# coreperf/rejit

Hardware: AMD Instinct MI355X
Metric: GB/s text scanned (regexdna 9 patterns, 50M-line input); matches/s alongside (higher is better)
Workload: dtype u8

## Files before the change

rejit_amd/csrc/plane_count.hip:

```cpp
#include <hip/hip_runtime.h>
#include <hip/hip_ext.h>

#include <cstdlib>

#include "exact_count.h"
#include "kernels.h"
#include "short_walk.h"
#include "stream_load.h"

namespace rejit_amd {

namespace {

constexpr int kWave = 64;
constexpr uint64_t kBlock = 2048;
constexpr uint32_t kPieceB = 1024;
constexpr uint32_t kStashWords = (2048 + 16) / 4;
#ifndef RJ_PC_RING
#define RJ_PC_RING 256
#endif
constexpr uint32_t kRing = RJ_PC_RING;

__device__ __forceinline__ int lane_id() { return static_cast<int>(threadIdx.x) & (kWave - 1); }

__device__ __forceinline__ uint32_t lanes_below(uint64_t mask) {
  return __builtin_amdgcn_mbcnt_hi(static_cast<uint32_t>(mask >> 32), __builtin_amdgcn_mbcnt_lo(static_cast<uint32_t>(mask), 0u));
}

__device__ __forceinline__ uint32_t from_lane_above(uint32_t v, uint32_t last) {
  return static_cast<uint32_t>(__builtin_amdgcn_update_dpp(static_cast<int>(last), static_cast<int>(v), 0x130, 0xF, 0xF, false));
}
__device__ __forceinline__ uint32_t from_lane_below(uint32_t v, uint32_t first) {
  return static_cast<uint32_t>(__builtin_amdgcn_update_dpp(static_cast<int>(first), static_cast<int>(v), 0x138, 0xF, 0xF, false));
}

template <int CTRL, int ROW_MASK>
__device__ __forceinline__ uint32_t dpp_or_zero(uint32_t x) {
  return static_cast<uint32_t>(__builtin_amdgcn_update_dpp(0, static_cast<int>(x), CTRL, ROW_MASK, 0xF, true));
}
__device__ __forceinline__ uint32_t wave_inclusive_sum(uint32_t x) {
  x += dpp_or_zero<0x111, 0xF>(x);
  x += dpp_or_zero<0x112, 0xF>(x);
  x += dpp_or_zero<0x114, 0xF>(x);
  x += dpp_or_zero<0x118, 0xF>(x);
  x += dpp_or_zero<0x142, 0xA>(x);
  x += dpp_or_zero<0x143, 0xC>(x);
  return x;
}

struct Consts {
  uint32_t cmask;
  uint32_t shift;
};

__device__ __forceinline__ uint32_t codes4(uint32_t d, const Consts& k) { return __builtin_amdgcn_udot4(d & k.cmask, 0x40100401u, 0u, false); }

__device__ __forceinline__ uint32_t codes16(const uint4& v, const Consts& k) {
  const uint32_t s = k.shift;
  return (codes4(v.x, k) >> s) | (codes4(v.y, k) << (8 - s)) | (codes4(v.z, k) << (16 - s)) | (codes4(v.w, k) << (24 - s));
}

struct Raw {
  uint4 a, b;
};

__device__ __forceinline__ void load_block(const uint8_t* block, uint32_t lane_off, Raw& r) {
  r.a = stream_load16(block + lane_off);
  r.b = stream_load16(block + lane_off + kPieceB);
}

__device__ __forceinline__ uint32_t guarded_dword(const uint8_t* text, uint64_t n, uint64_t at) {
  uint32_t v = 0;
#pragma unroll
  for (int k = 0; k < 4; k++)
    if (at + k < n) v |= static_cast<uint32_t>(text[at + k]) << (8 * k);
  return v;
}

template <int NB>
__device__ __forceinline__ uint32_t plane_test(uint32_t ta, uint32_t tb, uint32_t ha, uint32_t hb, const PlaneCountParams& a) {
  constexpr uint32_t kEven = 0x55555555u;
  const uint32_t L = (ta & kEven) | ((tb << 1) & ~kEven);
  const uint32_t H = ((ta >> 1) & kEven) | (tb & ~kEven);
  const uint32_t Ln = (ha & kEven) | ((hb << 1) & ~kEven);
  const uint32_t Hn = ((ha >> 1) & kEven) | (hb & ~kEven);
  register uint32_t q0 asm("v48") = ~(L | H);
  register uint32_t q1 asm("v49") = L & ~H;
  register uint32_t q2 asm("v50") = ~L & H;
  register uint32_t q3 asm("v51") = L & H;
  register uint32_t n0 asm("v52") = ~(Ln | Hn);
  register uint32_t n1 asm("v53") = Ln & ~Hn;
  register uint32_t n2 asm("v54") = ~Ln & Hn;
  register uint32_t n3 asm("v55") = Ln & Hn;
  uint32_t codes = ~a.mask_bits;
  asm volatile("" : "+s"(codes));
  auto code = [&](int b, int i) { return (codes >> (16 * b + 2 * i)) & 3u; };
  uint32_t E[8][NB], Z[NB], O[NB];
#pragma unroll
  for (int half = 0; half < 2; half++) {
    if (NB == 1) {
      if (half == 0) {
      asm volatile(
          "s_set_gpr_idx_on %[c00], 0x3\n"
          "v_mov_b32 %[e00], v48\n"
          "s_set_gpr_idx_idx %[c10]\n"
          "v_alignbit_b32 %[e10], v52, v48, 2\n"
          "s_set_gpr_idx_idx %[c20]\n"
          "v_alignbit_b32 %[e20], v52, v48, 4\n"
          "s_set_gpr_idx_idx %[c30]\n"
          "v_alignbit_b32 %[e30], v52, v48, 6\n"
          "s_set_gpr_idx_off\n"
          : [e00] "=&v"(E[0][0]), [e10] "=&v"(E[1][0]), [e20] "=&v"(E[2][0]), [e30] "=&v"(E[3][0])
          : [c00] "s"(code(0, 0)), [c10] "s"(code(0, 1)), [c20] "s"(code(0, 2)), [c30] "s"(code(0, 3)), "v"(q0), "v"(q1), "v"(q2), "v"(q3), "v"(n0), "v"(n1), "v"(n2), "v"(n3));
      } else {
      asm volatile(
          "s_set_gpr_idx_on %[c40], 0x3\n"
          "v_alignbit_b32 %[e40], v52, v48, 8\n"
          "s_set_gpr_idx_idx %[c50]\n"
          "v_alignbit_b32 %[e50], v52, v48, 10\n"
          "s_set_gpr_idx_idx %[c60]\n"
          "v_alignbit_b32 %[e60], v52, v48, 12\n"
          "s_set_gpr_idx_idx %[c70]\n"
          "v_alignbit_b32 %[e70], v52, v48, 14\n"
          "s_set_gpr_idx_off\n"
          : [e40] "=&v"(E[4][0]), [e50] "=&v"(E[5][0]), [e60] "=&v"(E[6][0]), [e70] "=&v"(E[7][0])
          : [c40] "s"(code(0, 4)), [c50] "s"(code(0, 5)), [c60] "s"(code(0, 6)), [c70] "s"(code(0, 7)), "v"(q0), "v"(q1), "v"(q2), "v"(q3), "v"(n0), "v"(n1), "v"(n2), "v"(n3));
      }
    } else {
      if (half == 0) {
      asm volatile(
          "s_set_gpr_idx_on %[c00], 0x3\n"
          "v_mov_b32 %[e00], v48\n"
          "s_set_gpr_idx_idx %[c01]\n"
          "v_mov_b32 %[e01], v48\n"
          "s_set_gpr_idx_idx %[c10]\n"
          "v_alignbit_b32 %[e10], v52, v48, 2\n"
          "s_set_gpr_idx_idx %[c11]\n"
          "v_alignbit_b32 %[e11], v52, v48, 2\n"
          "s_set_gpr_idx_idx %[c20]\n"
          "v_alignbit_b32 %[e20], v52, v48, 4\n"
          "s_set_gpr_idx_idx %[c21]\n"
          "v_alignbit_b32 %[e21], v52, v48, 4\n"
          "s_set_gpr_idx_idx %[c30]\n"
          "v_alignbit_b32 %[e30], v52, v48, 6\n"
          "s_set_gpr_idx_idx %[c31]\n"
          "v_alignbit_b32 %[e31], v52, v48, 6\n"
          "s_set_gpr_idx_off\n"
          : [e00] "=&v"(E[0][0]), [e01] "=&v"(E[0][1]), [e10] "=&v"(E[1][0]), [e11] "=&v"(E[1][1]), [e20] "=&v"(E[2][0]), [e21] "=&v"(E[2][1]), [e30] "=&v"(E[3][0]), [e31] "=&v"(E[3][1])
          : [c00] "s"(code(0, 0)), [c01] "s"(code(1, 0)), [c10] "s"(code(0, 1)), [c11] "s"(code(1, 1)), [c20] "s"(code(0, 2)), [c21] "s"(code(1, 2)), [c30] "s"(code(0, 3)), [c31] "s"(code(1, 3)), "v"(q0), "v"(q1), "v"(q2), "v"(q3), "v"(n0), "v"(n1), "v"(n2), "v"(n3));
      } else {
      asm volatile(
          "s_set_gpr_idx_on %[c40], 0x3\n"
          "v_alignbit_b32 %[e40], v52, v48, 8\n"
          "s_set_gpr_idx_idx %[c41]\n"
          "v_alignbit_b32 %[e41], v52, v48, 8\n"
          "s_set_gpr_idx_idx %[c50]\n"
          "v_alignbit_b32 %[e50], v52, v48, 10\n"
          "s_set_gpr_idx_idx %[c51]\n"
          "v_alignbit_b32 %[e51], v52, v48, 10\n"
          "s_set_gpr_idx_idx %[c60]\n"
          "v_alignbit_b32 %[e60], v52, v48, 12\n"
          "s_set_gpr_idx_idx %[c61]\n"
          "v_alignbit_b32 %[e61], v52, v48, 12\n"
          "s_set_gpr_idx_idx %[c70]\n"
          "v_alignbit_b32 %[e70], v52, v48, 14\n"
          "s_set_gpr_idx_idx %[c71]\n"
          "v_alignbit_b32 %[e71], v52, v48, 14\n"
          "s_set_gpr_idx_off\n"
          : [e40] "=&v"(E[4][0]), [e41] "=&v"(E[4][1]), [e50] "=&v"(E[5][0]), [e51] "=&v"(E[5][1]), [e60] "=&v"(E[6][0]), [e61] "=&v"(E[6][1]), [e70] "=&v"(E[7][0]), [e71] "=&v"(E[7][1])
          : [c40] "s"(code(0, 4)), [c41] "s"(code(1, 4)), [c50] "s"(code(0, 5)), [c51] "s"(code(1, 5)), [c60] "s"(code(0, 6)), [c61] "s"(code(1, 6)), [c70] "s"(code(0, 7)), [c71] "s"(code(1, 7)), "v"(q0), "v"(q1), "v"(q2), "v"(q3), "v"(n0), "v"(n1), "v"(n2), "v"(n3));
// ... 76 lines not shown

template <bool TOL>
__device__ __forceinline__ uint32_t general_test(uint32_t ta, uint32_t tb, uint32_t ha, uint32_t hb, const PlaneCountGParams& g) {
  constexpr uint32_t kEven = 0x55555555u;
  const uint32_t L = (ta & kEven) | ((tb << 1) & ~kEven);
  const uint32_t H = ((ta >> 1) & kEven) | (tb & ~kEven);
  const uint32_t Ln = (ha & kEven) | ((hb << 1) & ~kEven);
  const uint32_t Hn = ((ha >> 1) & kEven) | (hb & ~kEven);
  register uint32_t q0 asm("v48") = ~(L | H);
  register uint32_t q1 asm("v49") = L & ~H;
  register uint32_t q2 asm("v50") = ~L & H;
  register uint32_t q3 asm("v51") = L & H;
  register uint32_t q4 asm("v52") = ~0u;
  register uint32_t n0 asm("v56") = ~(Ln | Hn);
  register uint32_t n1 asm("v57") = Ln & ~Hn;
  register uint32_t n2 asm("v58") = ~Ln & Hn;
  register uint32_t n3 asm("v59") = Ln & Hn;
  register uint32_t n4 asm("v60") = ~0u;
  uint32_t c = 0;
#pragma clang loop unroll(disable)
  for (uint32_t b = 0; b < g.c.n_bases; b++) {
    const uint32_t* ix = g.idx[b];
    uint32_t e0, e1, e2, e3, e4, e5, e6, e7;
    asm volatile(
        "s_set_gpr_idx_on %[i0], 0x3\n"
        "v_mov_b32 %[e0], v48\n"
        "s_set_gpr_idx_idx %[i1]\n"
        "v_alignbit_b32 %[e1], v56, v48, 2\n"
        "s_set_gpr_idx_idx %[i2]\n"
        "v_alignbit_b32 %[e2], v56, v48, 4\n"
        "s_set_gpr_idx_idx %[i3]\n"
        "v_alignbit_b32 %[e3], v56, v48, 6\n"
        "s_set_gpr_idx_idx %[i4]\n"
        "v_alignbit_b32 %[e4], v56, v48, 8\n"
        "s_set_gpr_idx_idx %[i5]\n"
        "v_alignbit_b32 %[e5], v56, v48, 10\n"
        "s_set_gpr_idx_idx %[i6]\n"
        "v_alignbit_b32 %[e6], v56, v48, 12\n"
        "s_set_gpr_idx_idx %[i7]\n"
        "v_alignbit_b32 %[e7], v56, v48, 14\n"
        "s_set_gpr_idx_off\n"
        : [e0] "=&v"(e0), [e1] "=&v"(e1), [e2] "=&v"(e2), [e3] "=&v"(e3), [e4] "=&v"(e4), [e5] "=&v"(e5), [e6] "=&v"(e6), [e7] "=&v"(e7)
        : [i0] "s"(ix[0]), [i1] "s"(ix[1]), [i2] "s"(ix[2]), [i3] "s"(ix[3]), [i4] "s"(ix[4]), [i5] "s"(ix[5]), [i6] "s"(ix[6]), [i7] "s"(ix[7]), "v"(q0), "v"(q1), "v"(q2),
          "v"(q3), "v"(q4), "v"(n0), "v"(n1), "v"(n2), "v"(n3), "v"(n4));
    if (TOL) {
      uint32_t Z = e0, O = e0 | e1;
      Z &= e1;
      O = Z | (O & e2);
      Z &= e2;
      O = Z | (O & e3);
      Z &= e3;
      O = Z | (O & e4);
      Z &= e4;
      O = Z | (O & e5);
      Z &= e5;
      O = Z | (O & e6);
      Z &= e6;
      O = Z | (O & e7);
      c |= O;
    } else {
      const uint32_t z0 = e0 & e1 & e2, z1 = e3 & e4 & e5;
      c |= z0 & z1 & e6 & e7;
    }
  }
  return c;
}

}

template <int W, int MAXK, bool TOL>
struct GeneralShape {
  using Args = PlaneCountGParams;
  static constexpr uint32_t kFixedLen = 0;
  static constexpr bool kBlobInLds = true;
  static constexpr bool kList = false;
  static constexpr bool kCapture = false;
  __device__ static __forceinline__ void classify_bytes(const Args&, const uint32_t*, uint64_t, bool, uint32_t, uint32_t, uint32_t& mask) { mask = 0; }
  __device__ static __forceinline__ const PlaneCountParams& common(const Args& g) { return g.c; }
  __device__ static __forceinline__ uint32_t lmax(const Args& g) { return g.lmax; }
  __device__ static __forceinline__ uint32_t offset_of(const Args&, const uint32_t* blob, uint32_t p) {
    return reinterpret_cast<const ClassifyDesc*>(blob)[p].win_offset;
  }
  __device__ static __forceinline__ uint32_t test(uint32_t ta, uint32_t tb, uint32_t ha, uint32_t hb, const Args& g) { return general_test<TOL>(ta, tb, ha, hb, g); }
  __device__ static __forceinline__ void classify(const Args& g, const uint32_t* blob, uint64_t w, bool have, uint32_t& mask, Lens& lens) {
    const PlaneCountParams& a = g.c;
    const ClassifyDesc* desc = reinterpret_cast<const ClassifyDesc*>(blob);
    const uint32_t* tab = blob + g.desc_words;
    uint32_t lo = 0, hi = 0;
    if (have) {
      if (w + 8 <= a.n) {
        __builtin_memcpy(&lo, a.text + w, 4);
        __builtin_memcpy(&hi, a.text + w + 4, 4);
      } else {
        for (uint32_t q = 0; q < 8 && w + q < a.n; q++) {
          const uint32_t c = a.text[w + q];
          if (q < 4) lo |= c << (8 * q);
          else hi |= c << (8 * (q - 4));
        }
      }
    }
    uint32_t todo = 0;
    for (uint32_t p = 0; p < a.n_patterns; p++) {
      const ClassifyDesc& d = desc[p];
      const uint64_t s = w - d.win_offset;
      const bool ok = have && w >= d.win_offset && s >= a.sb && s < a.se && w + d.win_len <= a.n;
      bool win = false;
      for (uint32_t q = 0; q < d.n_windows; q++) win = win || ((((lo ^ d.v0[q]) & d.m0[q]) | ((hi ^ d.v1[q]) & d.m1[q])) == 0);
      todo |= (ok && win) ? 1u << p : 0u;
    }
    mask = 0;
    lens.w[0] = lens.w[1] = 0;
    while (__ballot(todo != 0) != 0) {
      const bool act = todo != 0;
      const uint32_t p = act ? static_cast<uint32_t>(__builtin_ctz(todo)) : 0u;
      todo &= todo - 1;
      const ClassifyDesc& d = desc[p];
      const uint32_t* t0 = tab + d.tab;
      const uint64_t s = w - d.win_offset;
      uint64_t t_lo = 0, t_hi = 0;
      if (act) rj_load16(a.text, a.n, s, &t_lo, &t_hi);
      const uint32_t avail = act ? (a.n - s < 16 ? static_cast<uint32_t>(a.n - s) : 16u) : 0u;
      uint32_t len = 0;
      bool found;
      if (W == 1 || d.n_words <= 1) found = short_longest_lds<1, MAXK>(t0, d, t_lo, t_hi, avail, &len);
      else found = short_longest_lds<W, MAXK>(t0, d, t_lo, t_hi, avail, &len);
      if (found && act && len != 0) {
        mask |= 1u << p;
        if (p < 12) lens.w[0] |= static_cast<uint64_t>(len) << (5 * p);
        else lens.w[1] |= static_cast<uint64_t>(len) << (5 * (p - 12));
      }
    }
  }
};

template <bool TOL>
struct GeneralListShape {
  using Args = PlaneListGParams;
  static constexpr uint32_t kFixedLen = 0;
  static constexpr bool kBlobInLds = false;
  static constexpr bool kList = true;
  static constexpr bool kCapture = false;
  __device__ static __forceinline__ void classify_bytes(const Args&, const uint32_t*, uint64_t, bool, uint32_t, uint32_t, uint32_t& mask) { mask = 0; }
  __device__ static __forceinline__ const PlaneCountParams& common(const Args& g) { return g.g.c; }
  __device__ static __forceinline__ uint32_t lmax(const Args& g) { return g.g.lmax; }
  __device__ static __forceinline__ uint32_t offset_of(const Args&, const uint32_t*, uint32_t) { return 0u; }
  __device__ static __forceinline__ uint32_t test(uint32_t ta, uint32_t tb, uint32_t ha, uint32_t hb, const Args& g) { return general_test<TOL>(ta, tb, ha, hb, g.g); }
  __device__ static __forceinline__ void classify(const Args&, const uint32_t*, uint64_t, bool, uint32_t& mask, Lens&) { mask = 0; }
};

namespace {

struct WaveState {
  uint32_t* ring;
  uint32_t* stash;
  uint32_t head, tail;
  uint32_t acc;
  uint32_t flags;
  uint32_t prev_rel, prev_valid;
  uint32_t* ends;
  uint64_t* list;
  uint32_t list_cap;
  uint64_t list_base;
};
constexpr uint32_t kNoEnd = 0xFFFFFFFFu;

template <bool LIST, bool CAPTURE>
__device__ __forceinline__ void push_block(WaveState& w, uint32_t hm, uint32_t rel_lane, uint32_t block_rel = 0, uint32_t slot = 0) {
  const uint64_t any = __ballot(hm != 0);
  if (any == 0) return;
  auto put = [&](uint32_t idx, uint32_t rel) {
    if (LIST) {
      if (idx < w.list_cap) w.list[idx] = w.list_base + rel;
    } else {
      w.ring[idx & (kRing - 1)] = rel;
      if (CAPTURE) {
        const uint32_t o = rel - block_rel;
        const uint32_t* sw = w.stash + slot * kStashWords + (o >> 2);
        const uint32_t s0 = sw[0], s1 = sw[1], s2 = sw[2];
        w.ring[kRing + (idx & (kRing - 1))] = __builtin_amdgcn_alignbyte(s1, s0, o & 3u);
        w.ring[2 * kRing + (idx & (kRing - 1))] = __builtin_amdgcn_alignbyte(s2, s1, o & 3u);
      }
    }
  };
  const uint32_t hm_a = hm & 0x55555555u, hm_b = hm & 0xAAAAAAAAu;
  const uint64_t several = __ballot((hm & (hm - 1)) != 0);
  if (several == 0) {
    const uint64_t any_a = __ballot(hm_a != 0);
    if (hm != 0) {
      const uint32_t bit = static_cast<uint32_t>(__builtin_ctz(hm));
      const uint32_t at = hm_a != 0 ? lanes_below(any_a) : static_cast<uint32_t>(__popcll(any_a)) + lanes_below(any & ~any_a);
      put(w.tail + at, rel_lane + (bit >> 1) + ((bit & 1u) ? kPieceB : 0u));
    }
    w.tail += static_cast<uint32_t>(__popcll(any));
    return;
  }
  const uint32_t c = __popc(hm_a) | (__popc(hm_b) << 16);
  const uint32_t inc = wave_inclusive_sum(c);
  const uint32_t tots = static_cast<uint32_t>(__builtin_amdgcn_readlane(static_cast<int>(inc), kWave - 1));
  const uint32_t tot_a = tots & 0xFFFFu, tot = tot_a + (tots >> 16);
  if (LIST || tot <= kRing) {
    const uint32_t before = inc - c;
    uint32_t idx = w.tail + (before & 0xFFFFu);
    for (uint32_t m = hm_a; m; m &= m - 1, idx++) put(idx, rel_lane + (static_cast<uint32_t>(__builtin_ctz(m)) >> 1));
    idx = w.tail + tot_a + (before >> 16);
    for (uint32_t m = hm_b; m; m &= m - 1, idx++) put(idx, rel_lane + kPieceB + (static_cast<uint32_t>(__builtin_ctz(m)) >> 1));
  }
  w.tail += tot;
}

template <class S>
__device__ __forceinline__ void classify_batch(WaveState& w, uint32_t m, const uint32_t* tab, const typename S::Args& g, uint64_t span_base) {
  const PlaneCountParams& a = S::common(g);
  const int lane = lane_id();
  const bool have = static_cast<uint32_t>(lane) < m;
  const uint32_t rel = w.ring[(w.head + static_cast<uint32_t>(lane)) & (kRing - 1)];
  uint32_t mask;
  Lens lens;
  if constexpr (S::kCapture) {
    const uint32_t lo = w.ring[kRing + ((w.head + static_cast<uint32_t>(lane)) & (kRing - 1))];
    const uint32_t hi = w.ring[2 * kRing + ((w.head + static_cast<uint32_t>(lane)) & (kRing - 1))];
    S::classify_bytes(g, tab, span_base + rel, have, lo, hi, mask);
  } else {
    S::classify(g, tab, span_base + rel, have, mask, lens);
  }
  const uint32_t before = from_lane_below(rel, w.prev_rel);
  const bool has_before = lane > 0 || w.prev_valid != 0;
  const bool close = have && has_before && (rel - before) < S::lmax(g);
  if (__ballot(close && mask != 0) != 0) {
    const uint32_t all_mask = mask;
    const uint32_t suspect = close ? all_mask : 0u;
    for (uint32_t p = 0; p < a.n_patterns; p++) {
      if (__ballot(((suspect >> p) & 1u) != 0) == 0) continue;
      const uint64_t all = __ballot(((all_mask >> p) & 1u) != 0);
      const uint32_t my_len = S::kFixedLen ? S::kFixedLen : len_of(lens, p);
      const uint32_t last_rel = w.ends[4 * p + 2], last_len = w.ends[4 * p + 3];
      uint32_t kept_end = w.ends[4 * p] == kNoEnd ? 0u : static_cast<uint32_t>(__builtin_amdgcn_readfirstlane(static_cast<int>(last_rel + last_len)));
      uint64_t kept = 0;
      for (uint64_t mm = all; mm != 0; mm &= mm - 1) {
        const int i = __builtin_ctzll(mm);
        const uint32_t wi = static_cast<uint32_t>(__builtin_amdgcn_readlane(static_cast<int>(rel), i));
        const uint32_t li = static_cast<uint32_t>(__builtin_amdgcn_readlane(static_cast<int>(my_len), i));
        if (wi >= kept_end) {
          kept |= 1ull << i;
          kept_end = wi + li;
        }
      }
      if ((((all & ~kept) >> lane) & 1ull) != 0) mask &= ~(1u << p);
    }
  }
  for (uint32_t p = 0; p < a.n_patterns; p++) {
    const uint64_t mine = __ballot(((mask >> p) & 1u) != 0);
    if (mine == 0) continue;
    if (lane == static_cast<int>(p)) w.acc += static_cast<uint32_t>(__popcll(mine));
    const int fl = __builtin_ctzll(mine), ll = 63 - __builtin_clzll(mine);
    const uint32_t my_len = S::kFixedLen ? S::kFixedLen : len_of(lens, p);
    const uint32_t first = static_cast<uint32_t>(__builtin_amdgcn_readlane(static_cast<int>(rel), fl));
    const uint32_t last = static_cast<uint32_t>(__builtin_amdgcn_readlane(static_cast<int>(rel), ll));
    const uint32_t first_len = S::kFixedLen ? S::kFixedLen : static_cast<uint32_t>(__builtin_amdgcn_readlane(static_cast<int>(my_len), fl));
    const uint32_t last_len = S::kFixedLen ? S::kFixedLen : static_cast<uint32_t>(__builtin_amdgcn_readlane(static_cast<int>(my_len), ll));
    if (lane == static_cast<int>(p)) {
      if (w.ends[4 * p] == kNoEnd) {
        w.ends[4 * p] = first;
        w.ends[4 * p + 1] = first_len;
      }
      w.ends[4 * p + 2] = last;
      w.ends[4 * p + 3] = last_len;
    }
  }
  w.prev_rel = static_cast<uint32_t>(__builtin_amdgcn_readlane(static_cast<int>(rel), static_cast<int>(m - 1)));
  w.prev_valid = 1;
  w.head += m;
}

template <class S>
__device__ __forceinline__ void check_span_start(WaveState& w, uint32_t m, const uint32_t* tab, const typename S::Args& g, uint64_t span_base) {
  const PlaneCountParams& a = S::common(g);
  const int lane = lane_id();
  const uint32_t reach = S::lmax(g) - 1u;
  const uint32_t rel = w.ring[(w.head + static_cast<uint32_t>(lane)) & (kRing - 1)];
  const bool near = static_cast<uint32_t>(lane) < m && static_cast<uint32_t>(lane) < reach && rel < reach;
  if (__ballot(near) == 0 || span_base == 0) return;
  uint32_t any[2] = {0, 0};
#pragma unroll
  for (int round = 0; round < 2; round++) {
    const uint64_t pos = round == 0 ? span_base + static_cast<uint64_t>(lane) - reach : span_base + rel;
    const bool mine = round == 0 ? (static_cast<uint32_t>(lane) < reach && span_base + static_cast<uint64_t>(lane) >= reach) : near;
    uint32_t mask;
    Lens lens;
    S::classify(g, tab, pos, mine, mask, lens);
    for (uint32_t p = 0; p < a.n_patterns; p++)
      if (__ballot(((mask >> p) & 1u) != 0) != 0) any[round] |= 1u << p;
  }
  if ((any[0] & any[1]) != 0) w.flags |= kPcConflict;
}

template <class S>
__device__ __forceinline__ void blocks_done(WaveState& w, const uint32_t* tab, const typename S::Args& g, uint64_t span_base, bool& first_batch) {
  const PlaneCountParams& a = S::common(g);
  if (w.tail - w.head > kRing) {
    w.flags |= kPcVoid;
    w.head = w.tail;
    return;
  }
  while (w.tail - w.head >= a.batch_at) {
    const uint32_t held = w.tail - w.head;
    const uint32_t m = held < 64u ? held : 64u;
    if (first_batch) check_span_start<S>(w, m, tab, g, span_base);
    first_batch = false;
    classify_batch<S>(w, m, tab, g, span_base);
  }
}

}

template <class S>
__global__ __launch_bounds__(256) void plane_count(typename S::Args g) {
  __shared__ __attribute__((aligned(16))) uint32_t table[kExactTabWords];
  extern __shared__ __attribute__((aligned(16))) uint32_t blob[];
  __shared__ uint32_t rings[4][kRing * (S::kCapture ? 3 : 1)];
  __shared__ __attribute__((aligned(16))) uint32_t stashes[4][S::kCapture ? 2 * kStashWords : 4];
  __shared__ uint32_t ends[4][4 * kExactMaxPatterns];
  __shared__ unsigned long long wave_bounds[4][kExactMaxPatterns][2];
  __shared__ uint32_t wave_counts[4][kExactMaxPatterns];
  __shared__ uint32_t wave_flags[4];
  const PlaneCountParams& a = S::common(g);
  const uint32_t* tab = S::kBlobInLds ? blob : table;
  const int lane = lane_id();
  const uint32_t wid = threadIdx.x >> 6;
  const uint32_t wave = __builtin_amdgcn_readfirstlane(static_cast<uint32_t>((static_cast<uint64_t>(blockIdx.x) * blockDim.x + threadIdx.x) >> 6));
  Consts k;
  k.shift = a.code_shift;
  k.cmask = 0x03030303u << a.code_shift;
  const uint32_t c0 = static_cast<uint32_t>(a.first_block) + wave * static_cast<uint32_t>(a.span_blocks) + (wave < a.span_extra ? wave : a.span_extra);
  const uint32_t c1 = c0 + static_cast<uint32_t>(a.span_blocks) + (wave < a.span_extra ? 1u : 0u);
  const uint32_t full = static_cast<uint32_t>(a.n / kBlock);
  uint32_t fast_end = full >= 1 ? full - 1 : 0;
  if (fast_end > c1) fast_end = c1;
  if (fast_end < c0) fast_end = c0;
  const uint64_t span_base = static_cast<uint64_t>(c0) * kBlock;
  WaveState w;
  w.ring = rings[wid];
  w.stash = stashes[wid];
  w.ends = ends[wid];
  w.head = w.tail = 0;
  w.acc = 0;
  w.flags = 0;
  w.prev_rel = w.prev_valid = 0;
  w.ends[lane] = kNoEnd;
  w.ends[lane + 64] = kNoEnd;
  w.list = nullptr;
  w.list_cap = 0;
  w.list_base = 0;
  if constexpr (S::kList) {
    if (wave == 0 && lane < kCntSize)
      for (uint32_t p = 0; p < g.n_zero; p++) g.zero_counters[p][lane] = 0;
    w.list = g.hits + static_cast<uint64_t>(wave) * g.region_cap;
    w.list_cap = g.region_cap;
    w.list_base = span_base - g.offset;
  }
  bool first_batch = true;

  const uint32_t last_own = fast_end > c0 ? fast_end - 1 : c0;
  auto blk = [&](uint32_t c) { return a.text + static_cast<uint64_t>(c < last_own ? c : last_own) * kBlock; };
  const uint32_t lane_rel = static_cast<uint32_t>(lane) * 16u;
  Raw ra, rb;
  uint2 behind{0, 0};
  uint32_t c = c0;
  auto stash_put = [&](uint32_t ci, const Raw& r) __attribute__((always_inline)) {
    if constexpr (S::kCapture) {
      uint32_t* sl = w.stash + (ci & 1u) * kStashWords;
      *reinterpret_cast<uint4*>(sl + lane * 4) = r.a;
      *reinterpret_cast<uint4*>(sl + kPieceB / 4 + lane * 4) = r.b;
    }
  };
  auto spill_put = [&](uint32_t ci, uint32_t x, uint32_t y) __attribute__((always_inline)) {
    if constexpr (S::kCapture) {
      if (lane == 0) *reinterpret_cast<uint2*>(w.stash + (ci & 1u) * kStashWords + kBlock / 4) = make_uint2(x, y);
    }
  };
  if (c < fast_end) {
    load_block(blk(c), lane_rel, ra);
    load_block(blk(c + 1), lane_rel, rb);
    behind = *reinterpret_cast<const uint2*>(a.text + static_cast<uint64_t>(fast_end) * kBlock);
  }
  if (S::kList) {
  } else if (S::kBlobInLds) {
    const uint4* src = reinterpret_cast<const uint4*>(a.table);
    uint4* dst = reinterpret_cast<uint4*>(blob);
    for (uint32_t i = threadIdx.x; i < a.table_words / 4; i += blockDim.x) dst[i] = src[i];
  } else {
    for (uint32_t i = threadIdx.x; i < kExactTabWords; i += blockDim.x) table[i] = a.table[i];
  }
  __syncthreads();
  if (c < fast_end) {
    uint32_t xa = codes16(ra.a, k), xb = codes16(ra.b, k);
    stash_put(c, ra);
    if (S::kCapture) __builtin_amdgcn_sched_barrier(0);
    load_block(blk(c + 2), lane_rel, ra);
    const uint32_t behind_codes = (codes4(behind.x, k) >> k.shift) | (codes4(behind.y, k) << (8 - k.shift));
    while (c + 1 < fast_end) {
      const uint32_t ya = codes16(rb.a, k), yb = codes16(rb.b, k);
      asm volatile("" ::"v"(ya), "v"(yb));
      stash_put(c + 1, rb);
      spill_put(c, rb.a.x, rb.a.y);
      if (S::kCapture) __builtin_amdgcn_sched_barrier(0);
      if (c + 3 <= last_own) load_block(blk(c + 3), lane_rel, rb);
      {
        const uint32_t ha = from_lane_above(xa, static_cast<uint32_t>(__builtin_amdgcn_readfirstlane(static_cast<int>(xb))));
        const uint32_t hb = from_lane_above(xb, static_cast<uint32_t>(__builtin_amdgcn_readfirstlane(static_cast<int>(ya))));
        const uint32_t hm = S::test(xa, xb, ha, hb, g);
        push_block<S::kList, S::kCapture>(w, hm, (c - c0) * static_cast<uint32_t>(kBlock) + lane_rel, (c - c0) * static_cast<uint32_t>(kBlock), c & 1u);
      }
      __builtin_amdgcn_sched_barrier(0);
      xa = codes16(ra.a, k);
      xb = codes16(ra.b, k);
      asm volatile("" ::"v"(xa), "v"(xb));
      if (c + 2 < fast_end) {
        stash_put(c + 2, ra);
        spill_put(c + 1, ra.a.x, ra.a.y);
      } else {
        spill_put(c + 1, behind.x, behind.y);
      }
      if (S::kCapture) __builtin_amdgcn_sched_barrier(0);
      if (c + 4 <= last_own) load_block(blk(c + 4), lane_rel, ra);
      {
        const uint32_t next0 = c + 2 == fast_end ? behind_codes : static_cast<uint32_t>(__builtin_amdgcn_readfirstlane(static_cast<int>(xa)));
        const uint32_t ha = from_lane_above(ya, static_cast<uint32_t>(__builtin_amdgcn_readfirstlane(static_cast<int>(yb))));
        const uint32_t hb = from_lane_above(yb, next0);
        const uint32_t hm = S::test(ya, yb, ha, hb, g);
        push_block<S::kList, S::kCapture>(w, hm, (c + 1 - c0) * static_cast<uint32_t>(kBlock) + lane_rel, (c + 1 - c0) * static_cast<uint32_t>(kBlock), (c + 1) & 1u);
      }
      __builtin_amdgcn_sched_barrier(0);
      c += 2;
      if (!S::kList && w.tail - w.head >= a.batch_at) blocks_done<S>(w, tab, g, span_base, first_batch);
    }
    if (c + 1 == fast_end) {
      const uint32_t ha = from_lane_above(xa, static_cast<uint32_t>(__builtin_amdgcn_readfirstlane(static_cast<int>(xb))));
      const uint32_t hb = from_lane_above(xb, static_cast<uint32_t>(__builtin_amdgcn_readfirstlane(static_cast<int>(behind_codes))));
      const uint32_t hm = S::test(xa, xb, ha, hb, g);
      spill_put(c, behind.x, behind.y);
      push_block<S::kList, S::kCapture>(w, hm, (c - c0) * static_cast<uint32_t>(kBlock) + lane_rel, (c - c0) * static_cast<uint32_t>(kBlock), c & 1u);
      c++;
    }
    if (!S::kList) blocks_done<S>(w, tab, g, span_base, first_batch);
  }
  for (; c < c1; c++) {
    const uint64_t at = static_cast<uint64_t>(c) * kBlock + lane_rel, bt = at + kPieceB;
    uint4 va, vb;
    va.x = guarded_dword(a.text, a.n, at);
    va.y = guarded_dword(a.text, a.n, at + 4);
    va.z = guarded_dword(a.text, a.n, at + 8);
    va.w = guarded_dword(a.text, a.n, at + 12);
    vb.x = guarded_dword(a.text, a.n, bt);
    vb.y = guarded_dword(a.text, a.n, bt + 4);
    vb.z = guarded_dword(a.text, a.n, bt + 8);
    vb.w = guarded_dword(a.text, a.n, bt + 12);
    const uint32_t g0 = guarded_dword(a.text, a.n, at + 16), g1 = guarded_dword(a.text, a.n, at + 20);
    const uint32_t h0 = guarded_dword(a.text, a.n, bt + 16), h1 = guarded_dword(a.text, a.n, bt + 20);
    const uint32_t ha = (codes4(g0, k) >> k.shift) | (codes4(g1, k) << (8 - k.shift));
    const uint32_t hb = (codes4(h0, k) >> k.shift) | (codes4(h1, k) << (8 - k.shift));
    const uint32_t hm = S::test(codes16(va, k), codes16(vb, k), ha, hb, g);
    if (!S::kList && w.tail - w.head > kRing - 64u) blocks_done<S>(w, tab, g, span_base, first_batch);
    if constexpr (S::kCapture) {
      Raw gr;
      gr.a = va;
      gr.b = vb;
      stash_put(c, gr);
      const uint64_t nb = (static_cast<uint64_t>(c) + 1) * kBlock;
      spill_put(c, guarded_dword(a.text, a.n, nb), guarded_dword(a.text, a.n, nb + 4));
    }
    push_block<S::kList, S::kCapture>(w, hm, (c - c0) * static_cast<uint32_t>(kBlock) + lane_rel, (c - c0) * static_cast<uint32_t>(kBlock), c & 1u);
  }
  if constexpr (S::kList) {
    if (lane == 0) g.hit_counts[wave] = w.tail;
    return;
  }
  if (w.tail - w.head > kRing) {
    w.flags |= kPcVoid;
    w.head = w.tail;
  }
  while (w.tail != w.head) {
    const uint32_t held = w.tail - w.head;
    const uint32_t m = held < 64u ? held : 64u;
    if (first_batch) check_span_start<S>(w, m, tab, g, span_base);
    first_batch = false;
    classify_batch<S>(w, m, tab, g, span_base);
  }
  if (lane < kExactMaxPatterns) {
    const bool real = lane < static_cast<int>(a.n_patterns);
    wave_counts[wid][lane] = real ? w.acc : 0u;
    const uint32_t ef = w.ends[4 * lane], efl = w.ends[4 * lane + 1], el = w.ends[4 * lane + 2], ell = w.ends[4 * lane + 3];
    const uint64_t off = real ? S::offset_of(g, tab, static_cast<uint32_t>(lane)) : 0u;
    wave_bounds[wid][lane][0] = ef != kNoEnd ? ((span_base + ef - off) | (static_cast<unsigned long long>(efl) << kPcLenShift)) : kPcNone;
    wave_bounds[wid][lane][1] = ef != kNoEnd ? ((span_base + el - off) | (static_cast<unsigned long long>(ell) << kPcLenShift)) : kPcNone;
  }
  if (lane == 0) wave_flags[wid] = w.flags;
  __syncthreads();
  if (wid != 0 || lane >= kExactMaxPatterns) return;
  uint32_t v = wave_counts[0][lane] + wave_counts[1][lane] + wave_counts[2][lane] + wave_counts[3][lane];
  if (lane == kExactMaxPatterns - 1) v = wave_flags[0] | wave_flags[1] | wave_flags[2] | wave_flags[3];
  a.wg_rows[static_cast<uint64_t>(blockIdx.x) * kExactMaxPatterns + lane] = v;
  if (lane < static_cast<int>(a.n_patterns) && v != 0) {
    unsigned long long first = kPcNone, last = kPcNone;
#pragma unroll
    for (int q = 3; q >= 0; q--)
      if (wave_bounds[q][lane][0] != kPcNone) first = wave_bounds[q][lane][0];
#pragma unroll
    for (int q = 0; q < 4; q++)
      if (wave_bounds[q][lane][1] != kPcNone) last = wave_bounds[q][lane][1];
    *reinterpret_cast<ulonglong2*>(a.wg_bounds + (static_cast<uint64_t>(blockIdx.x) * kExactMaxPatterns + lane) * 2) = ulonglong2{first, last};
  }
}

constexpr uint32_t kFinishBatch = 8;
__global__ __launch_bounds__(256, 8) void plane_count_finish(PlaneCountParams a, uint32_t n_wg) {
  __shared__ unsigned long long part[32][kExactMaxPatterns];
  __shared__ uint32_t part_first[32][kExactMaxPatterns], part_last[32][kExactMaxPatterns];
  __shared__ uint32_t is_last;
  const uint32_t p4 = threadIdx.x & 7u, q = threadIdx.x >> 3;
  const uint32_t per = (n_wg + gridDim.x - 1) / gridDim.x;
  const uint32_t r_lo = blockIdx.x * per, r_hi = r_lo + per < n_wg ? r_lo + per : n_wg;
  uint32_t sum[4] = {0, 0, 0, 0};
  uint32_t first_row[4] = {0, 0, 0, 0}, last_row[4] = {0, 0, 0, 0};
  const uint4* rows = reinterpret_cast<const uint4*>(a.wg_rows);
  for (uint32_t r = r_lo + q; r < r_hi; r += 32 * kFinishBatch) {
    uint4 v[kFinishBatch];
#pragma unroll
    for (uint32_t i = 0; i < kFinishBatch; i++) {
      const uint32_t rr = r + 32 * i;
      v[i] = rows[static_cast<uint64_t>(rr < r_hi ? rr : r) * 8 + p4];
      if (rr >= r_hi) v[i] = uint4{0, 0, 0, 0};
    }
#pragma unroll
    for (uint32_t i = 0; i < kFinishBatch; i++) {
      const uint32_t rr1 = r + 32 * i + 1;
      const uint32_t c[4] = {v[i].x, v[i].y, v[i].z, v[i].w};
      sum[0] += v[i].x;
      sum[1] += v[i].y;
      sum[2] += v[i].z;
      sum[3] = p4 == 7 ? (sum[3] | v[i].w) : (sum[3] + v[i].w);
#pragma unroll
      for (int k = 0; k < 4; k++) {
        first_row[k] = (c[k] != 0 && first_row[k] == 0) ? rr1 : first_row[k];
        last_row[k] = c[k] != 0 ? rr1 : last_row[k];
      }
    }
  }
#pragma unroll
  for (int i = 0; i < 4; i++) {
    part[q][4 * p4 + i] = sum[i];
    part_first[q][4 * p4 + i] = first_row[i];
    part_last[q][4 * p4 + i] = last_row[i];
  }
  __syncthreads();
  const uint32_t lane = threadIdx.x & 63u, wave_id = threadIdx.x >> 6;
  if (wave_id == 0) {
    if (lane < kExactMaxPatterns) {
      unsigned long long t = 0;
      uint32_t f = 0, l = 0;
#pragma unroll 4
      for (uint32_t i = 0; i < 32; i++) {
        t = lane == kExactMaxPatterns - 1 ? (t | part[i][lane]) : (t + part[i][lane]);
        const uint32_t pf = part_first[i][lane], pl = part_last[i][lane];
        f = pf != 0 && (f == 0 || pf < f) ? pf : f;
        l = pl > l ? pl : l;
      }
      unsigned long long* g = a.acc + kPcGroupRows + blockIdx.x * 96;
      __hip_atomic_store(&g[lane], t, __ATOMIC_RELAXED, __HIP_MEMORY_SCOPE_AGENT);
      __hip_atomic_store(&g[32 + lane], static_cast<unsigned long long>(f), __ATOMIC_RELAXED, __HIP_MEMORY_SCOPE_AGENT);
      __hip_atomic_store(&g[64 + lane], static_cast<unsigned long long>(l), __ATOMIC_RELAXED, __HIP_MEMORY_SCOPE_AGENT);
    }
    if (lane == 0) {
      const unsigned long long t = __hip_atomic_fetch_add(&a.acc[kPcTicket], 1ull, __ATOMIC_ACQ_REL, __HIP_MEMORY_SCOPE_AGENT);
      is_last = t + 1 == gridDim.x ? 1u : 0u;
      if (t + 1 == gridDim.x) __hip_atomic_store(&a.acc[kPcTicket], 0ull, __ATOMIC_RELAXED, __HIP_MEMORY_SCOPE_AGENT);
    }
  }
  __syncthreads();
  if (!is_last || threadIdx.x >= kExactMaxPatterns) return;
  const uint32_t p = threadIdx.x;
  unsigned long long total = 0;
  uint32_t f = 0, l = 0;
#pragma unroll 2
  for (uint32_t g = 0; g < gridDim.x; g++) {
    const unsigned long long* row = a.acc + kPcGroupRows + g * 96;
    const unsigned long long v = __hip_atomic_load(&row[p], __ATOMIC_RELAXED, __HIP_MEMORY_SCOPE_AGENT);
    const uint32_t pf = static_cast<uint32_t>(__hip_atomic_load(&row[32 + p], __ATOMIC_RELAXED, __HIP_MEMORY_SCOPE_AGENT));
    const uint32_t pl = static_cast<uint32_t>(__hip_atomic_load(&row[64 + p], __ATOMIC_RELAXED, __HIP_MEMORY_SCOPE_AGENT));
    total = p == kExactMaxPatterns - 1 ? (total | v) : (total + v);
    f = pf != 0 && (f == 0 || pf < f) ? pf : f;
    l = pl > l ? pl : l;
  }
  if (p == kExactMaxPatterns - 1) a.host_out[kPcHostFlags] = total;
  if (p >= a.n_patterns) return;
  unsigned long long first = kPcNone, last = kPcNone;
  if (total != 0 && f != 0) {
    first = a.wg_bounds[(static_cast<uint64_t>(f - 1) * kExactMaxPatterns + p) * 2];
    last = a.wg_bounds[(static_cast<uint64_t>(l - 1) * kExactMaxPatterns + p) * 2 + 1];
  }
  a.host_out[kPcHostCount + p] = total;
  a.host_out[kPcHostBounds + 2 * p] = first;
  a.host_out[kPcHostBounds + 2 * p + 1] = last;
  a.acc[kPcBounds + 2 * p] = first;
  a.acc[kPcBounds + 2 * p + 1] = last;
  a.acc[kPcTotals + p] = total;
}

__global__ void bounds_rows_counts_kernel(BoundsParams a, const unsigned long long* acc, int64_t offset, int first_round, int64_t* rows) {
  const int p = threadIdx.x;
  if (p >= a.n_lists) return;
  uint64_t n = a.count[p];
  int64_t fb = -1, fe = -1, lb = -1, le = -1;
  if (a.spans[p]) {
    const uint64_t* r = a.spans[p];
    if (n) {
      fb = static_cast<int64_t>(r[0]) + offset;
      fe = static_cast<int64_t>(r[1]) + offset;
      lb = static_cast<int64_t>(r[2 * (n - 1)]) + offset;
      le = static_cast<int64_t>(r[2 * (n - 1) + 1]) + offset;
    }
  } else {
    n = acc[kPcTotals + p];
    if (n) {
      const unsigned long long f = acc[kPcBounds + 2 * p], l = acc[kPcBounds + 2 * p + 1];
// ... 57 lines not shown
```

Baseline: 50390.

## Capture match windows from registers and deepen capture-path prefetch to four buffers

In the capture variant, the per-wave LDS stash of each 2KB block is removed. Each hit's 8-byte window is now built directly from the lane's loaded registers, with the following dwords fetched from the neighbouring lane via DPP. The capture loop is rewritten as a rotating 3- or 4-buffer prefetch pipeline with compile-time unrolled steps. This removes LDS stores and loads per block and reduces LDS footprint, at the cost of more VGPRs for the extra in-flight buffers and per-hit register selects.

```diff
diff --git a/rejit_amd/csrc/plane_count.hip b/rejit_amd/csrc/plane_count.hip
--- a/rejit_amd/csrc/plane_count.hip
+++ b/rejit_amd/csrc/plane_count.hip
@@ -2,6 +2,7 @@
 #include <hip/hip_ext.h>
 
 #include <cstdlib>
+#include <type_traits>
 
 #include "exact_count.h"
 #include "kernels.h"
@@ -15,7 +16,11 @@
 constexpr int kWave = 64;
 constexpr uint64_t kBlock = 2048;
 constexpr uint32_t kPieceB = 1024;
-constexpr uint32_t kStashWords = (2048 + 16) / 4;
+#ifndef RJ_PC_BUFS
+#define RJ_PC_BUFS 4
+#endif
+constexpr int kCapBufs = RJ_PC_BUFS;
+static_assert(kCapBufs == 3 || kCapBufs == 4, "the capture loop is written out for three or four buffers");
 #ifndef RJ_PC_RING
 #define RJ_PC_RING 256
 #endif
@@ -398,7 +403,6 @@
 
 struct WaveState {
   uint32_t* ring;
-  uint32_t* stash;
   uint32_t head, tail;
   uint32_t acc;
   uint32_t flags;
@@ -410,21 +414,39 @@
 };
 constexpr uint32_t kNoEnd = 0xFFFFFFFFu;
 
-template <bool LIST, bool CAPTURE>
-__device__ __forceinline__ void push_block(WaveState& w, uint32_t hm, uint32_t rel_lane, uint32_t block_rel = 0, uint32_t slot = 0) {
+struct Windows {
+  uint4 a, b;
+  uint32_t na0, na1, nb0, nb1;
+};
+
+__device__ __forceinline__ void window_bytes(const Windows& v, uint32_t bit, uint32_t& lo, uint32_t& hi) {
+  const bool pb = (bit & 1u) != 0;
+  const uint32_t k = bit >> 1, q = k >> 2;
+  const uint32_t d0 = pb ? v.b.x : v.a.x, d1 = pb ? v.b.y : v.a.y, d2 = pb ? v.b.z : v.a.z, d3 = pb ? v.b.w : v.a.w;
+  const uint32_t d4 = pb ? v.nb0 : v.na0, d5 = pb ? v.nb1 : v.na1;
+  const uint32_t s0 = q == 0 ? d0 : q == 1 ? d1 : q == 2 ? d2 : d3;
+  const uint32_t s1 = q == 0 ? d1 : q == 1 ? d2 : q == 2 ? d3 : d4;
+  const uint32_t s2 = q == 0 ? d2 : q == 1 ? d3 : q == 2 ? d4 : d5;
+  lo = __builtin_amdgcn_alignbyte(s1, s0, k & 3u);
+  hi = __builtin_amdgcn_alignbyte(s2, s1, k & 3u);
+}
+
+template <bool LIST, bool CAPTURE, class F = int>
+__device__ __forceinline__ void push_block(WaveState& w, uint32_t hm, uint32_t rel_lane, F&& windows = 0) {
   const uint64_t any = __ballot(hm != 0);
   if (any == 0) return;
-  auto put = [&](uint32_t idx, uint32_t rel) {
+  Windows win{};
+  if constexpr (CAPTURE) win = windows();
+  auto put = [&](uint32_t idx, uint32_t rel, uint32_t bit) {
     if (LIST) {
       if (idx < w.list_cap) w.list[idx] = w.list_base + rel;
     } else {
       w.ring[idx & (kRing - 1)] = rel;
       if (CAPTURE) {
-        const uint32_t o = rel - block_rel;
-        const uint32_t* sw = w.stash + slot * kStashWords + (o >> 2);
-        const uint32_t s0 = sw[0], s1 = sw[1], s2 = sw[2];
-        w.ring[kRing + (idx & (kRing - 1))] = __builtin_amdgcn_alignbyte(s1, s0, o & 3u);
-        w.ring[2 * kRing + (idx & (kRing - 1))] = __builtin_amdgcn_alignbyte(s2, s1, o & 3u);
+        uint32_t lo, hi;
+        window_bytes(win, bit, lo, hi);
+        w.ring[kRing + (idx & (kRing - 1))] = lo;
+        w.ring[2 * kRing + (idx & (kRing - 1))] = hi;
       }
     }
   };
@@ -435,7 +457,7 @@
     if (hm != 0) {
       const uint32_t bit = static_cast<uint32_t>(__builtin_ctz(hm));
       const uint32_t at = hm_a != 0 ? lanes_below(any_a) : static_cast<uint32_t>(__popcll(any_a)) + lanes_below(any & ~any_a);
-      put(w.tail + at, rel_lane + (bit >> 1) + ((bit & 1u) ? kPieceB : 0u));
+      put(w.tail + at, rel_lane + (bit >> 1) + ((bit & 1u) ? kPieceB : 0u), bit);
     }
     w.tail += static_cast<uint32_t>(__popcll(any));
     return;
@@ -447,9 +469,9 @@
   if (LIST || tot <= kRing) {
     const uint32_t before = inc - c;
     uint32_t idx = w.tail + (before & 0xFFFFu);
-    for (uint32_t m = hm_a; m; m &= m - 1, idx++) put(idx, rel_lane + (static_cast<uint32_t>(__builtin_ctz(m)) >> 1));
+    for (uint32_t m = hm_a; m; m &= m - 1, idx++) put(idx, rel_lane + (static_cast<uint32_t>(__builtin_ctz(m)) >> 1), static_cast<uint32_t>(__builtin_ctz(m)));
     idx = w.tail + tot_a + (before >> 16);
-    for (uint32_t m = hm_b; m; m &= m - 1, idx++) put(idx, rel_lane + kPieceB + (static_cast<uint32_t>(__builtin_ctz(m)) >> 1));
+    for (uint32_t m = hm_b; m; m &= m - 1, idx++) put(idx, rel_lane + kPieceB + (static_cast<uint32_t>(__builtin_ctz(m)) >> 1), static_cast<uint32_t>(__builtin_ctz(m)));
   }
   w.tail += tot;
 }
@@ -564,7 +586,6 @@
   __shared__ __attribute__((aligned(16))) uint32_t table[kExactTabWords];
   extern __shared__ __attribute__((aligned(16))) uint32_t blob[];
   __shared__ uint32_t rings[4][kRing * (S::kCapture ? 3 : 1)];
-  __shared__ __attribute__((aligned(16))) uint32_t stashes[4][S::kCapture ? 2 * kStashWords : 4];
   __shared__ uint32_t ends[4][4 * kExactMaxPatterns];
   __shared__ unsigned long long wave_bounds[4][kExactMaxPatterns][2];
   __shared__ uint32_t wave_counts[4][kExactMaxPatterns];
@@ -586,7 +607,6 @@
   const uint64_t span_base = static_cast<uint64_t>(c0) * kBlock;
   WaveState w;
   w.ring = rings[wid];
-  w.stash = stashes[wid];
   w.ends = ends[wid];
   w.head = w.tail = 0;
   w.acc = 0;
@@ -609,86 +629,136 @@
   const uint32_t last_own = fast_end > c0 ? fast_end - 1 : c0;
   auto blk = [&](uint32_t c) { return a.text + static_cast<uint64_t>(c < last_own ? c : last_own) * kBlock; };
   const uint32_t lane_rel = static_cast<uint32_t>(lane) * 16u;
-  Raw ra, rb;
   uint2 behind{0, 0};
   uint32_t c = c0;
-  auto stash_put = [&](uint32_t ci, const Raw& r) __attribute__((always_inline)) {
-    if constexpr (S::kCapture) {
-      uint32_t* sl = w.stash + (ci & 1u) * kStashWords;
-      *reinterpret_cast<uint4*>(sl + lane * 4) = r.a;
-      *reinterpret_cast<uint4*>(sl + kPieceB / 4 + lane * 4) = r.b;
-    }
+  auto stage_tables = [&]() __attribute__((always_inline)) {
+    if (S::kList) {
+    } else if (S::kBlobInLds) {
+      const uint4* src = reinterpret_cast<const uint4*>(a.table);
+      uint4* dst = reinterpret_cast<uint4*>(blob);
+      for (uint32_t i = threadIdx.x; i < a.table_words / 4; i += blockDim.x) dst[i] = src[i];
+    } else {
+      for (uint32_t i = threadIdx.x; i < kExactTabWords; i += blockDim.x) table[i] = a.table[i];
+    }
+    __syncthreads();
   };
-  auto spill_put = [&](uint32_t ci, uint32_t x, uint32_t y) __attribute__((always_inline)) {
-    if constexpr (S::kCapture) {
-      if (lane == 0) *reinterpret_cast<uint2*>(w.stash + (ci & 1u) * kStashWords + kBlock / 4) = make_uint2(x, y);
-    }
-  };
-  if (c < fast_end) {
-    load_block(blk(c), lane_rel, ra);
-    load_block(blk(c + 1), lane_rel, rb);
-    behind = *reinterpret_cast<const uint2*>(a.text + static_cast<uint64_t>(fast_end) * kBlock);
-  }
-  if (S::kList) {
-  } else if (S::kBlobInLds) {
-    const uint4* src = reinterpret_cast<const uint4*>(a.table);
-    uint4* dst = reinterpret_cast<uint4*>(blob);
-    for (uint32_t i = threadIdx.x; i < a.table_words / 4; i += blockDim.x) dst[i] = src[i];
+  if constexpr (!S::kCapture) {
+    Raw ra, rb;
+    if (c < fast_end) {
+      load_block(blk(c), lane_rel, ra);
+      load_block(blk(c + 1), lane_rel, rb);
+      behind = *reinterpret_cast<const uint2*>(a.text + static_cast<uint64_t>(fast_end) * kBlock);
+    }
+    stage_tables();
+    if (c < fast_end) {
+      uint32_t xa = codes16(ra.a, k), xb = codes16(ra.b, k);
+      load_block(blk(c + 2), lane_rel, ra);
+      const uint32_t behind_codes = (codes4(behind.x, k) >> k.shift) | (codes4(behind.y, k) << (8 - k.shift));
+      while (c + 1 < fast_end) {
+        const uint32_t ya = codes16(rb.a, k), yb = codes16(rb.b, k);
+        asm volatile("" ::"v"(ya), "v"(yb));
+        if (c + 3 <= last_own) load_block(blk(c + 3), lane_rel, rb);
+        {
+          const uint32_t ha = from_lane_above(xa, static_cast<uint32_t>(__builtin_amdgcn_readfirstlane(static_cast<int>(xb))));
+          const uint32_t hb = from_lane_above(xb, static_cast<uint32_t>(__builtin_amdgcn_readfirstlane(static_cast<int>(ya))));
+          const uint32_t hm = S::test(xa, xb, ha, hb, g);
+          push_block<S::kList, false>(w, hm, (c - c0) * static_cast<uint32_t>(kBlock) + lane_rel);
+        }
+        __builtin_amdgcn_sched_barrier(0);
+        xa = codes16(ra.a, k);
+        xb = codes16(ra.b, k);
+        asm volatile("" ::"v"(xa), "v"(xb));
+        if (c + 4 <= last_own) load_block(blk(c + 4), lane_rel, ra);
+        {
+          const uint32_t next0 = c + 2 == fast_end ? behind_codes : static_cast<uint32_t>(__builtin_amdgcn_readfirstlane(static_cast<int>(xa)));
+          const uint32_t ha = from_lane_above(ya, static_cast<uint32_t>(__builtin_amdgcn_readfirstlane(static_cast<int>(yb))));
+          const uint32_t hb = from_lane_above(yb, next0);
+          const uint32_t hm = S::test(ya, yb, ha, hb, g);
+          push_block<S::kList, false>(w, hm, (c + 1 - c0) * static_cast<uint32_t>(kBlock) + lane_rel);
+        }
+        __builtin_amdgcn_sched_barrier(0);
+        c += 2;
+        if (!S::kList && w.tail - w.head >= a.batch_at) blocks_done<S>(w, tab, g, span_base, first_batch);
+      }
+      if (c + 1 == fast_end) {
+        const uint32_t ha = from_lane_above(xa, static_cast<uint32_t>(__builtin_amdgcn_readfirstlane(static_cast<int>(xb))));
+        const uint32_t hb = from_lane_above(xb, static_cast<uint32_t>(__builtin_amdgcn_readfirstlane(static_cast<int>(behind_codes))));
+        const uint32_t hm = S::test(xa, xb, ha, hb, g);
+        push_block<S::kList, false>(w, hm, (c - c0) * static_cast<uint32_t>(kBlock) + lane_rel);
+        c++;
+      }
+      if (!S::kList) blocks_done<S>(w, tab, g, span_base, first_batch);
+    }
   } else {
-    for (uint32_t i = threadIdx.x; i < kExactTabWords; i += blockDim.x) table[i] = a.table[i];
-  }
-  __syncthreads();
-  if (c < fast_end) {
-    uint32_t xa = codes16(ra.a, k), xb = codes16(ra.b, k);
-    stash_put(c, ra);
-    if (S::kCapture) __builtin_amdgcn_sched_barrier(0);
-    load_block(blk(c + 2), lane_rel, ra);
-    const uint32_t behind_codes = (codes4(behind.x, k) >> k.shift) | (codes4(behind.y, k) << (8 - k.shift));
-    while (c + 1 < fast_end) {
-      const uint32_t ya = codes16(rb.a, k), yb = codes16(rb.b, k);
-      asm volatile("" ::"v"(ya), "v"(yb));
-      stash_put(c + 1, rb);
-      spill_put(c, rb.a.x, rb.a.y);
-      if (S::kCapture) __builtin_amdgcn_sched_barrier(0);
-      if (c + 3 <= last_own) load_block(blk(c + 3), lane_rel, rb);
-      {
-        const uint32_t ha = from_lane_above(xa, static_cast<uint32_t>(__builtin_amdgcn_readfirstlane(static_cast<int>(xb))));
-        const uint32_t hb = from_lane_above(xb, static_cast<uint32_t>(__builtin_amdgcn_readfirstlane(static_cast<int>(ya))));
-        const uint32_t hm = S::test(xa, xb, ha, hb, g);
-        push_block<S::kList, S::kCapture>(w, hm, (c - c0) * static_cast<uint32_t>(kBlock) + lane_rel, (c - c0) * static_cast<uint32_t>(kBlock), c & 1u);
-      }
-      __builtin_amdgcn_sched_barrier(0);
-      xa = codes16(ra.a, k);
-      xb = codes16(ra.b, k);
-      asm volatile("" ::"v"(xa), "v"(xb));
-      if (c + 2 < fast_end) {
-        stash_put(c + 2, ra);
-        spill_put(c + 1, ra.a.x, ra.a.y);
-      } else {
-        spill_put(c + 1, behind.x, behind.y);
-      }
-      if (S::kCapture) __builtin_amdgcn_sched_barrier(0);
-      if (c + 4 <= last_own) load_block(blk(c + 4), lane_rel, ra);
-      {
-        const uint32_t next0 = c + 2 == fast_end ? behind_codes : static_cast<uint32_t>(__builtin_amdgcn_readfirstlane(static_cast<int>(xa)));
-        const uint32_t ha = from_lane_above(ya, static_cast<uint32_t>(__builtin_amdgcn_readfirstlane(static_cast<int>(yb))));
-        const uint32_t hb = from_lane_above(yb, next0);
-        const uint32_t hm = S::test(ya, yb, ha, hb, g);
-        push_block<S::kList, S::kCapture>(w, hm, (c + 1 - c0) * static_cast<uint32_t>(kBlock) + lane_rel, (c + 1 - c0) * static_cast<uint32_t>(kBlock), (c + 1) & 1u);
-      }
-      __builtin_amdgcn_sched_barrier(0);
-      c += 2;
-      if (!S::kList && w.tail - w.head >= a.batch_at) blocks_done<S>(w, tab, g, span_base, first_batch);
-    }
-    if (c + 1 == fast_end) {
-      const uint32_t ha = from_lane_above(xa, static_cast<uint32_t>(__builtin_amdgcn_readfirstlane(static_cast<int>(xb))));
-      const uint32_t hb = from_lane_above(xb, static_cast<uint32_t>(__builtin_amdgcn_readfirstlane(static_cast<int>(behind_codes))));
-      const uint32_t hm = S::test(xa, xb, ha, hb, g);
-      spill_put(c, behind.x, behind.y);
-      push_block<S::kList, S::kCapture>(w, hm, (c - c0) * static_cast<uint32_t>(kBlock) + lane_rel, (c - c0) * static_cast<uint32_t>(kBlock), c & 1u);
-      c++;
-    }
-    if (!S::kList) blocks_done<S>(w, tab, g, span_base, first_batch);
+    Raw r[kCapBufs] = {};
+    if (c < fast_end) {
+      load_block(blk(c), lane_rel, r[0]);
+      if (c + 1 <= last_own) load_block(blk(c + 1), lane_rel, r[1]);
+      if (c + 2 <= last_own) load_block(blk(c + 2), lane_rel, r[2]);
+      if constexpr (kCapBufs > 3)
+        if (c + 3 <= last_own) load_block(blk(c + 3), lane_rel, r[kCapBufs - 1]);
+      behind = *reinterpret_cast<const uint2*>(a.text + static_cast<uint64_t>(fast_end) * kBlock);
+    }
+    stage_tables();
+    if (c < fast_end) {
+      uint32_t xa = codes16(r[0].a, k), xb = codes16(r[0].b, k);
+      const uint32_t behind_codes = (codes4(behind.x, k) >> k.shift) | (codes4(behind.y, k) << (8 - k.shift));
+      auto step = [&](auto U, auto TAIL) __attribute__((always_inline)) {
+        constexpr int u = decltype(U)::value, un = (u + 1) % kCapBufs;
+        constexpr bool tail = decltype(TAIL)::value;
+        const uint32_t j = c + static_cast<uint32_t>(u);
+        const bool last = tail && j + 1 == fast_end;
+        const uint32_t ya = codes16(r[un].a, k), yb = codes16(r[un].b, k);
+        asm volatile("" ::"v"(ya), "v"(yb));
+        {
+          const uint32_t next0 = last ? behind_codes : static_cast<uint32_t>(__builtin_amdgcn_readfirstlane(static_cast<int>(ya)));
+          const uint32_t ha = from_lane_above(xa, static_cast<uint32_t>(__builtin_amdgcn_readfirstlane(static_cast<int>(xb))));
+          const uint32_t hb = from_lane_above(xb, next0);
+          const uint32_t hm = S::test(xa, xb, ha, hb, g);
+          push_block<false, true>(w, hm, (j - c0) * static_cast<uint32_t>(kBlock) + lane_rel, [&]() {
+            const uint32_t n0 = last ? behind.x : r[un].a.x, n1 = last ? behind.y : r[un].a.y;
+            Windows v;
+            v.a = r[u].a;
+            v.b = r[u].b;
+            v.na0 = from_lane_above(v.a.x, static_cast<uint32_t>(__builtin_amdgcn_readfirstlane(static_cast<int>(v.b.x))));
+            v.na1 = from_lane_above(v.a.y, static_cast<uint32_t>(__builtin_amdgcn_readfirstlane(static_cast<int>(v.b.y))));
+            v.nb0 = from_lane_above(v.b.x, static_cast<uint32_t>(__builtin_amdgcn_readfirstlane(static_cast<int>(n0))));
+            v.nb1 = from_lane_above(v.b.y, static_cast<uint32_t>(__builtin_amdgcn_readfirstlane(static_cast<int>(n1))));
+            return v;
+          });
+        }
+        __builtin_amdgcn_sched_barrier(0);
+        if (!tail) load_block(a.text + static_cast<uint64_t>(j + kCapBufs) * kBlock, lane_rel, r[u]);
+        else if (j + kCapBufs <= last_own) load_block(blk(j + kCapBufs), lane_rel, r[u]);
+        __builtin_amdgcn_sched_barrier(0);
+        xa = ya;
+        xb = yb;
+      };
+      using std::integral_constant;
+      constexpr integral_constant<bool, false> kBody{};
+      constexpr integral_constant<bool, true> kTail{};
+      while (c + 2 * kCapBufs <= fast_end) {
+        step(integral_constant<int, 0>{}, kBody);
+        step(integral_constant<int, 1>{}, kBody);
+        if (kCapBufs == 4 && w.tail - w.head >= a.batch_at) blocks_done<S>(w, tab, g, span_base, first_batch);
+        step(integral_constant<int, 2>{}, kBody);
+        if constexpr (kCapBufs > 3) step(integral_constant<int, kCapBufs - 1>{}, kBody);
+        c += kCapBufs;
+        if (w.tail - w.head >= a.batch_at) blocks_done<S>(w, tab, g, span_base, first_batch);
+      }
+      while (c < fast_end) {
+        step(integral_constant<int, 0>{}, kTail);
+        if (c + 1 < fast_end) step(integral_constant<int, 1>{}, kTail);
+        if (kCapBufs == 4 && w.tail - w.head >= a.batch_at) blocks_done<S>(w, tab, g, span_base, first_batch);
+        if (c + 2 < fast_end) step(integral_constant<int, 2>{}, kTail);
+        if constexpr (kCapBufs > 3)
+          if (c + 3 < fast_end) step(integral_constant<int, kCapBufs - 1>{}, kTail);
+        c += kCapBufs;
+        if (w.tail - w.head >= a.batch_at) blocks_done<S>(w, tab, g, span_base, first_batch);
+      }
+      c = fast_end;
+      blocks_done<S>(w, tab, g, span_base, first_batch);
+    }
   }
   for (; c < c1; c++) {
     const uint64_t at = static_cast<uint64_t>(c) * kBlock + lane_rel, bt = at + kPieceB;
@@ -708,14 +778,10 @@
     const uint32_t hm = S::test(codes16(va, k), codes16(vb, k), ha, hb, g);
     if (!S::kList && w.tail - w.head > kRing - 64u) blocks_done<S>(w, tab, g, span_base, first_batch);
     if constexpr (S::kCapture) {
-      Raw gr;
-      gr.a = va;
-      gr.b = vb;
-      stash_put(c, gr);
-      const uint64_t nb = (static_cast<uint64_t>(c) + 1) * kBlock;
-      spill_put(c, guarded_dword(a.text, a.n, nb), guarded_dword(a.text, a.n, nb + 4));
-    }
-    push_block<S::kList, S::kCapture>(w, hm, (c - c0) * static_cast<uint32_t>(kBlock) + lane_rel, (c - c0) * static_cast<uint32_t>(kBlock), c & 1u);
+      push_block<false, true>(w, hm, (c - c0) * static_cast<uint32_t>(kBlock) + lane_rel, [&]() { return Windows{va, vb, g0, g1, h0, h1}; });
+    } else {
+      push_block<S::kList, false>(w, hm, (c - c0) * static_cast<uint32_t>(kBlock) + lane_rel);
+    }
   }
   if constexpr (S::kList) {
     if (lane == 0) g.hit_counts[wave] = w.tail;
```

Result: slower. 49780 (-1.2%).
